# tomka/mitsuba-renderer

Hardware: AMD Instinct MI355X
Metric: Msamples/s (higher is better)
Workload: dtype f32; 1 GPU; C3 1M-tri Cornell: 1024000-tri displaced walls TriMesh + 20480-tri dielectric icosphere + area light, path maxDepth=16 rrDepth=10, 1024x1024, ldsampler 64 spp per GPU (64 per frame, weak scaling), box filter; triangles=1044482, kd_nodes=551229, kd_indices=1101661, parallelism=ImageBlock tiles, morton(tx, ty) % 1 + one RCCL film reduce per frame

## Files before the change

mitsuba-renderer_amd/csrc/api.cpp:

```cpp
#include "host.h"
#include "kernels.h"
#include "devmath.h"
#include "ctx.h"
#include <algorithm>
#include <cstdarg>
#include <cstdio>
#include <cstring>
#include <cstdlib>
#include <cmath>

using namespace mg;

namespace mg {
thread_local std::string g_lastError;

int fail(mtsgpu_ctx *ctx, int code, const char *fmt, ...) {
	char buf[512];
	va_list ap; va_start(ap, fmt); vsnprintf(buf, sizeof(buf), fmt, ap); va_end(ap);
	g_lastError = buf;
	if (ctx) ctx->error = buf;
	return code;
}
}

// ... 41 lines not shown
	c->q.tune_refill = c->tuning.count("refill_min") ? 1u : 0u;
	c->q.tune_batch = (uint32_t) get("batch", 0);
	c->q.tune_dyn_div = (uint32_t) get("dyn_div", 0);
	c->q.tune_blocks_per_cu = (uint32_t) get("blocks_per_cu", 0);
	c->q.tune_plain_below = (uint32_t) get("plain_below", 0);
	c->q.tune_dyn_min_rounds = (uint32_t) get("dyn_min_rounds", 0);
	c->q.bin_hits = c->binHits;
}

int filmWidth(const mtsgpu_ctx *c) { return c->cam.film_width > 0 ? c->cam.film_width : c->cam.width; }
int filmHeight(const mtsgpu_ctx *c) { return c->cam.film_height > 0 ? c->cam.film_height : c->cam.height; }

uint32_t tileMorton(uint32_t tx, uint32_t ty) {
	uint32_t m = 0;
	for (int b = 0; b < 16; ++b)
		m |= ((tx >> b) & 1u) << (2 * b) | ((ty >> b) & 1u) << (2 * b + 1);
	return m;
}

bool samplerHasTables(const mtsgpu_ctx *c) {
	return c->samplerKind == MTSGPU_SAMPLER_LD_KEYED || c->samplerKind == MTSGPU_SAMPLER_STRATIFIED_KEYED;
}

constexpr size_t kBytesPerPath = kPathSlots * 16 + 3 * 16 + (size_t) (kNumBins * (4 + 16) * 5 / 4) + 2 * (4 + 32) + 4 + 4;
uint64_t defaultMaxPaths(mtsgpu_ctx *c) {
	uint64_t paths = 72ull << 20;
	size_t freeB = 0, totalB = 0;
	if (hipMemGetInfo(&freeB, &totalB) == hipSuccess) {
		uint64_t avail = (uint64_t) freeB + (uint64_t) c->pathCap * kBytesPerPath;
		if (c->filmStats && !c->statVar) avail -= std::min<uint64_t>(avail, 16ull * (uint64_t) c->cam.width * (uint64_t) c->cam.height);
		paths = std::min<uint64_t>(paths, std::max<uint64_t>(1ull << 16, avail * 6 / 10 / kBytesPerPath));
	}
	return paths;
}

int ensurePaths(mtsgpu_ctx *c, size_t cap) {
	if (cap <= c->pathCap)
		return 0;
	freeAll(c->pathAllocs);
	c->pathCap = 0;
	cap = (cap + 255) & ~(size_t) 255;
	auto &o = c->pathAllocs;
	int rc = 0;
	rc |= devAlloc(c, &c->paths.base, cap * kPathSlots, o);
	rc |= devAlloc(c, &c->paths.shq_o, cap, o); rc |= devAlloc(c, &c->paths.shq_d, cap, o); rc |= devAlloc(c, &c->paths.shq_nee, cap, o);
	const unsigned gridBlocksMax = c->nCUs * kTraceBlocksPerCuMax;
	const size_t segCap = cap / kBinShards + cap / (4 * kBinShards) + (size_t) kTraceBlock * (gridBlocksMax / kBinShards + 2);
	rc |= devAlloc(c, &c->q.bins_base, segCap * kBinShards * kNumBins, o);
	rc |= devAlloc(c, &c->binHits, segCap * kBinShards * kNumBins, o);
	applyTuning(c);
	c->q.bin_stride = (uint32_t) (segCap * kBinShards);
	if (segCap * kBinShards > 0xFFFFFFFFull) return fail(c, MTSGPU_EINVAL, "pass too large");
	c->q.bin_seg_cap = (uint32_t) segCap;
	rc |= devAlloc(c, &c->queueA, cap, o); rc |= devAlloc(c, &c->queueB, cap, o);
	for (int k = 0; k < 2; ++k) { rc |= devAlloc(c, &c->rayqA[k], cap, o); rc |= devAlloc(c, &c->rayqB[k], cap, o); }
	rc |= devAlloc(c, &c->q.shadow, cap, o);
	rc |= devAlloc(c, &c->counterSets, (size_t) kCounterSets * kNumCounters * kCounterStride, o);
	rc |= devAlloc(c, &c->viewsDev, kNumBins, o);
	rc |= devAlloc(c, &c->devStats, kNumDevStats, o);
	rc |= devAlloc(c, &c->q.trace_counts, kNumTraceCounts, o);
	rc |= devAlloc(c, &c->spillClosest, (size_t) gridBlocksMax * kTraceBlock * trace_spill_levels(), o);
	rc |= devAlloc(c, &c->spillShadow, (size_t) gridBlocksMax * kTraceBlock * trace_spill_levels(), o);
	if (rc) return rc;
	c->q.counters = c->counterSets; c->q.spill = c->spillClosest; c->q.dev_stats = nullptr;
	c->q.spill_stride = gridBlocksMax * kTraceBlock;
	c->q.n_cus = c->nCUs; c->q.force_static = 0;
	applyTuning(c);
	HIPCHK(c, hipMemset(c->q.trace_counts, 0, kNumTraceCounts * sizeof(unsigned long long)));
	c->q.rec = c->q.rec_len = nullptr; c->q.rec_cap = 0;
	c->pathCap = cap;
	return 0;
}

template <typename T> int ensureBuf(mtsgpu_ctx *c, T **p, size_t *cap, size_t need) {
	if (need <= *cap) return 0;
	if (*p) (void) hipFree(*p);
	*p = nullptr; *cap = 0;
	void *raw = nullptr;
	HIPCHK(c, hipMalloc(&raw, need * sizeof(T)));
	*p = static_cast<T *>(raw); *cap = need;
	return 0;
}

int ensureTableWork(mtsgpu_ctx *c, size_t nSlots, uint32_t spp) {
	int rc = ensureBuf(c, &c->ldState, &c->ldStateCap, nSlots); if (rc) return rc;
	return ensureBuf(c, &c->ldScratch, &c->ldScratchCap, ld_table_scratch_entries((uint32_t) nSlots, spp, c->ldDepth));
}

DConfig makeConfig(const mtsgpu_ctx *c, bool slotPerPath) {
	DConfig cfg{};
	std::memcpy(cfg.r2c, c->cam.raster_to_camera, sizeof(cfg.r2c));
	std::memcpy(cfg.c2w, c->cam.camera_to_world, sizeof(cfg.c2w));
	cfg.near_clip = c->cam.near_clip; cfg.far_clip = c->cam.far_clip;
	cfg.aperture_radius = c->cam.aperture_radius; cfg.focus_depth = c->cam.focus_depth; cfg.camera_kind = c->cam.kind;
	cfg.width = c->cam.width; cfg.height = c->cam.height;
	cfg.crop_x = c->cam.crop_offset_x; cfg.crop_y = c->cam.crop_offset_y;
	cfg.pix_w = filmWidth(c); cfg.pix_off = 0;
	cfg.max_depth = c->maxDepth; cfg.rr_depth = c->rrDepth; cfg.strict_normals = c->strictNormals;
	cfg.integrator = c->integrator; cfg.n_lum = c->nLumSamples; cfg.n_bsdf = c->nBsdfSamples;
	cfg.weight_bsdf = 1 / (float) c->nBsdfSamples; cfg.weight_lum = 1 / (float) c->nLumSamples;
	cfg.frac_bsdf = c->nBsdfSamples / (float) (c->nLumSamples + c->nBsdfSamples);
	cfg.frac_lum = c->nLumSamples / (float) (c->nLumSamples + c->nBsdfSamples);
	cfg.sampler_kind = c->samplerKind;
	cfg.spp = effectiveSpp(c); cfg.ld_depth = c->ldDepth; cfg.seed = c->seed;
	cfg.strat_res = 1; while ((uint32_t) cfg.strat_res * (uint32_t) cfg.strat_res < cfg.spp) ++cfg.strat_res;
	cfg.slot_per_path = slotPerPath ? 1 : 0;
// ... 93 lines not shown
			}
			views[b].prefix[kBinShards] = acc;
		}
		if (attempt == 0 && c->tuning.count("test_retry") && c->tuning["test_retry"]) overflow = true;
		if (!overflow) return 0;
		c->stats.bin_overflow_retries++;
	}
	return fail(c, MTSGPU_EHIP, "internal: bin segment overflow with static dealing");
}

int runDirectRounds(mtsgpu_ctx *c, const DConfig &cfg0, uint32_t nPaths, volatile const int *cancel) {
	hipStream_t s = c->stream;
	DConfig cfg = cfg0;
	const size_t counterBytes = kNumCounters * kCounterStride * sizeof(uint32_t);
	auto timedTrace = [&](int mode, bool bin, const uint32_t *queue, uint32_t n, bool coherent) -> int {
		hipEvent_t *ev = c->timeKernels ? nextTraceEvents(c, mode == 1 ? 2 : 0) : nullptr;
		if (ev) HIPCHK(c, hipEventRecord(ev[0], s));
		launch_trace(s, mode, c->countTraversal, bin, c->dsc, c->paths, c->q, queue, n, coherent);
		if (ev) HIPCHK(c, hipEventRecord(ev[1], s));
		HIPCHK(c, hipGetLastError());
		c->stats.trace_launches++;
		return 0;
	};
	HIPCHK(c, hipMemsetAsync(c->q.counters, 0, counterBytes, s));
	c->q.next = c->queueB;
	BinView views[kNumBins];
	RayQueuesOff rqOff{ c };
	rayQueues(c, c->queueA, nullptr);
	int rc = traceAndBin(c, c->queueA, nPaths, true, views); if (rc) return rc;
	rayQueues(c, nullptr, nullptr);
	c->stats.rays_closest += nPaths;
	auto shadeRound = [&](int mode, int index, bool withTerminal) -> int {
		hipEvent_t *sev = c->timeKernels ? nextEventPair(c, c->shadeEvents, c->shadeEvUsed) : nullptr;
		HIPCHK(c, hipMemsetAsync(c->q.counters, 0, counterBytes, s));
		if (sev) HIPCHK(c, hipEventRecord(sev[0], s));
		cfg.dr_mode = mode; cfg.dr_index = index;
		for (int b = 0; b < (withTerminal ? kNumBins : kNumBsdfTypes); ++b)
			launch_shade(s, b, c->dsc, c->paths, cfg, c->q, views[b], nullptr, 0, nullptr, c->dcol, c->dtex, c->dtan);
		if (sev) HIPCHK(c, hipEventRecord(sev[1], s));
		HIPCHK(c, hipGetLastError());
		return readCounters(c);
	};
	for (int j = 0; j < std::max(1, c->nLumSamples); ++j) {
		if (cancel && *cancel) return fail(c, MTSGPU_ECANCEL, "render cancelled");
		rc = shadeRound(1, j, j == 0); if (rc) return rc;
		const uint32_t nShadow = c->hostCounters[kShadowWord];
// ... 30 lines not shown
}

int runBouncesDevice(mtsgpu_ctx *c, const DConfig &cfg, uint32_t nPaths, volatile const int *cancel) {
	hipStream_t s1 = c->stream, s2 = c->stream2;
	const size_t setBytes = (size_t) kNumCounters * kCounterStride * sizeof(uint32_t);
	HIPCHK(c, hipMemsetAsync(c->counterSets, 0, kCounterSets * setBytes, s1));
	c->q.dev_stats = c->devStats;
	c->devStatsUsed = true;
	const int limit = cfg.integrator == 1 ? 2 : (cfg.max_depth > 0 ? cfg.max_depth : 0x7FFFFFFF);
	const int chunk = (int) tuningOr(c, "chunk", 8);
	uint32_t *cur = c->queueA, *nxt = c->queueB;
	uint32_t upper = nPaths;
	bool shadowPending = false;
	int b = 0;
	struct Restore {
		mtsgpu_ctx *c; hipStream_t s2; const bool &pending;
		~Restore() {
			if (pending) (void) hipStreamSynchronize(s2);
			c->q.dev_stats = nullptr; c->q.counters = c->counterSets; c->q.spill = c->spillClosest;
		}
	} restore{ c, s2, shadowPending };
	RayQueuesOff rqOff{ c };
	c->q.nee_parked = tuningOr(c, "nee_parked", 1) != 0 ? 1u : 0u;
	auto timed = [&](std::vector<std::pair<hipEvent_t, hipEvent_t>> &pool, size_t &used, hipStream_t s, int which, int cls = -1) -> int {
		if (!c->timeKernels) return 0;
		hipEvent_t *ev = which == 0 ? (cls >= 0 ? nextTraceEvents(c, cls) : nextEventPair(c, pool, used)) : &pool[used - 1].first;
		if (!ev) return fail(c, MTSGPU_EHIP, "hipEventCreate failed");
		HIPCHK(c, hipEventRecord(ev[which], s));
		return 0;
	};
	while (b < limit && upper > 0) {
		if (cancel && *cancel) return fail(c, MTSGPU_ECANCEL, "render cancelled");
		const int end = (int) std::min<long long>((long long) b + chunk, limit);
		for (; b < end; ++b) {
			uint32_t *set = counterSet(c, b), *prev = counterSet(c, b - 1);
			c->q.counters = set; c->q.next = nxt; c->q.spill = c->spillClosest;
			rayQueues(c, cur, nxt);
			int rc = timed(c->traceEvents, c->traceEvUsed, s1, 0, b == 0 ? 1 : 0); if (rc) return rc;
			launch_trace(s1, 0, c->countTraversal, true, c->dsc, c->paths, c->q, cur, upper, b == 0,
			             b == 0 ? nullptr : prev + (size_t) kNextWord);
			rc = timed(c->traceEvents, c->traceEvUsed, s1, 1); if (rc) return rc;
			if (shadowPending) HIPCHK(c, hipStreamWaitEvent(s1, c->evShadow[(b - 1) & 1], 0));
			rc = timed(c->shadeEvents, c->shadeEvUsed, s1, 0); if (rc) return rc;
			launch_prep(s1, set, prev, c->viewsDev, c->q.bin_seg_cap, c->devStats);
			if (cfg.dr_mode == 0 && tuningOr(c, "shade_fused", 1) != 0) {
				launch_shade_all(s1, c->dsc, c->paths, cfg, c->q, c->viewsDev, c->binMask & kShadeAllBins, upper, c->dcol, c->dtex, c->dtan);
// ... 40 lines not shown
	unsigned long long h[kNumDevStats];
	HIPCHK(c, hipMemcpy(h, c->devStats, sizeof(h), hipMemcpyDeviceToHost));
	c->stats.rays_closest += h[kStatClosest]; c->stats.rays_shadow += h[kStatShadow]; c->stats.trace_launches += h[kStatLaunches];
	if (h[kStatOverflow]) return fail(c, MTSGPU_EHIP, "internal: bin segment overflow in a device-driven frame");
	return 0;
}

int runBounces(mtsgpu_ctx *c, const DConfig &cfg, uint32_t nPaths, volatile const int *cancel) {
	c->q.counters = c->counterSets; c->q.spill = c->spillClosest; c->q.dev_stats = nullptr;
	if (cfg.integrator == 1 && (cfg.n_lum > 1 || cfg.n_bsdf > 1))
		return runDirectRounds(c, cfg, nPaths, cancel);
	{
		const long sf = tuningOr(c, "sync_free", -1);
		if (sf == 1 || (sf < 0 && nPaths <= (8u << 20)))
			return runBouncesDevice(c, cfg, nPaths, cancel);
	}
	uint32_t nQ = nPaths;
	uint32_t *cur = c->queueA, *nxt = c->queueB;
	bool first = true;
	hipStream_t s = c->stream;
	const size_t setBytes = (size_t) kNumCounters * kCounterStride * sizeof(uint32_t);
	RayQueuesOff rqOff{ c };
	c->q.nee_parked = tuningOr(c, "nee_parked", 1) != 0 ? 1u : 0u;
	for (int b = 0; nQ > 0; ++b) {
		if (cancel && *cancel)
			return fail(c, MTSGPU_ECANCEL, "render cancelled");
		c->q.counters = counterSet(c, b); c->q.spill = c->spillClosest;
		HIPCHK(c, hipMemsetAsync(c->q.counters, 0, setBytes, s));
		c->q.next = nxt;
		rayQueues(c, cur, nxt);
		BinView views[kNumBins];
		int rc = traceAndBin(c, cur, nQ, first, views); if (rc) return rc;
		c->stats.rays_closest += nQ;
		hipEvent_t *sev = c->timeKernels ? nextEventPair(c, c->shadeEvents, c->shadeEvUsed) : nullptr;
		if (sev) HIPCHK(c, hipEventRecord(sev[0], s));
		for (int bin = 0; bin < kNumBins; ++bin)
			launch_shade(s, bin, c->dsc, c->paths, cfg, c->q, views[bin], nullptr, 0, nullptr, c->dcol, c->dtex, c->dtan);
		if (sev) HIPCHK(c, hipEventRecord(sev[1], s));
		HIPCHK(c, hipGetLastError());
		rc = readCounters(c); if (rc) return rc;
		const uint32_t nNext = c->hostCounters[kNextWord], nShadow = c->hostCounters[kShadowWord];
		if (nShadow) {
			DQueues q2 = c->q; q2.spill = c->spillShadow;
			c->lastPass.shadowMax = std::max(c->lastPass.shadowMax, nShadow);
			hipEvent_t *ev2 = c->timeKernels ? nextTraceEvents(c, 2) : nullptr;
			if (ev2) HIPCHK(c, hipEventRecord(ev2[0], s));
// ... 135 lines not shown
		    || hipMemcpy(c->primes, primes.data(), primes.size() * sizeof(uint16_t), hipMemcpyHostToDevice) != hipSuccess) {
			mtsgpu_destroy(c); return fail(nullptr, MTSGPU_EHIP, "prime table upload failed");
		}
	}
	*out = c;
	return 0;
}

void mtsgpu_destroy(mtsgpu_ctx *c) {
	if (!c) return;
	(void) hipSetDevice(c->device);
	(void) hipDeviceSynchronize();
	freeAll(c->sceneAllocs); freeAll(c->colorAllocs); freeAll(c->texAllocs); freeAll(c->pathAllocs);
	if (c->ownFilm && c->film) (void) hipFree(c->film);
	if (c->pixelList) (void) hipFree(c->pixelList);
	if (c->ldScr) (void) hipFree(c->ldScr);
	if (c->ldPerm) (void) hipFree(c->ldPerm);
	if (c->ldState) (void) hipFree(c->ldState);
	if (c->ldScratch) (void) hipFree(c->ldScratch);
	if (c->arrScr) (void) hipFree(c->arrScr);
	if (c->arrPerm) (void) hipFree(c->arrPerm);
	if (c->arrPts) (void) hipFree(c->arrPts);
	if (c->primSave) (void) hipFree(c->primSave);
	if (c->primes) (void) hipFree(c->primes);
	if (c->pathLen) (void) hipFree(c->pathLen);
	if (c->explicitSamples) (void) hipFree(c->explicitSamples);
	if (c->filtValues) (void) hipFree(c->filtValues);
	if (c->statVar) (void) hipFree(c->statVar);
	if (c->statN) (void) hipFree(c->statN);
	if (c->tileMeta) (void) hipFree(c->tileMeta);
	if (c->blocks) (void) hipFree(c->blocks);
	if (c->hostCounters) (void) hipHostFree(c->hostCounters);
	for (auto &e : c->traceEvents) { (void) hipEventDestroy(e.first); (void) hipEventDestroy(e.second); }
	for (auto &e : c->shadeEvents) { (void) hipEventDestroy(e.first); (void) hipEventDestroy(e.second); }
	if (c->ownStream && c->stream) (void) hipStreamDestroy(c->stream);
	if (c->stream2) (void) hipStreamDestroy(c->stream2);
	for (hipEvent_t e : { c->evShade[0], c->evShade[1], c->evShadow[0], c->evShadow[1], c->evCount }) if (e) (void) hipEventDestroy(e);
	delete c;
}

int mtsgpu_set_stream(mtsgpu_ctx *c, void *hip_stream) {
	if (!c) return fail(nullptr, MTSGPU_EINVAL, "null context");
	if (c->ownStream && c->stream) { (void) hipStreamSynchronize(c->stream); (void) hipStreamDestroy(c->stream); }
	if (hip_stream) { c->stream = (hipStream_t) hip_stream; c->ownStream = false; }
	else { HIPCHK(c, hipStreamCreate(&c->stream)); c->ownStream = true; }
	return 0;
// ... 882 lines not shown
	hipEvent_t e0 = nullptr, e1 = nullptr;
	auto cleanup = [&]() {
		for (uint32_t *p : { rec, recLen, order, tr, batchLen, sink }) if (p) (void) hipFree(p);
		if (tmp) (void) hipFree(tmp);
		if (e0) (void) hipEventDestroy(e0);
		if (e1) (void) hipEventDestroy(e1);
		c->q.rec = c->q.rec_len = nullptr; c->q.rec_cap = 0;
	};
	#define RR_CHK(expr) do { hipError_t e_ = (expr); if (e_ != hipSuccess) { cleanup(); \
		return fail(c, MTSGPU_EHIP, "%s failed: %s (%s:%d)", #expr, hipGetErrorString(e_), __FILE__, __LINE__); } } while (0)
	RR_CHK(hipMalloc((void **) &rec, (size_t) n * cap * 4)); RR_CHK(hipMalloc((void **) &recLen, (size_t) n * 4));
	RR_CHK(hipMalloc((void **) &order, (size_t) n * 4)); RR_CHK(hipMalloc((void **) &tr, (size_t) nBatches * cap * 64 * 4));
	RR_CHK(hipMalloc((void **) &batchLen, (size_t) nBatches * 4)); RR_CHK(hipMalloc((void **) &sink, 4));
	RR_CHK(hipEventCreate(&e0)); RR_CHK(hipEventCreate(&e1));
	const size_t counterBytes = kNumCounters * kCounterStride * sizeof(uint32_t);
	c->q.counters = c->counterSets; c->q.spill = mode == 1 ? c->spillShadow : c->spillClosest; c->q.dev_stats = nullptr;
	c->q.next = c->queueB;
	if (kind == 1) {
		launch_generate(s, c->dsc, c->paths, lp.cfg, c->pixelList + lp.base, lp.nSlots, nullptr, lp.nPaths, c->queueA);
		RR_CHK(hipGetLastError());
		c->lastPass.valid = false;
	}
	if (kind == 2) {
		RR_CHK(hipMalloc((void **) &tmp, (size_t) n * 3 * sizeof(float4)));
		launch_gather_strided(s, tmp, c->paths.shq_o, n, stride); launch_gather_strided(s, tmp + n, c->paths.shq_d, n, stride);
		launch_gather_strided(s, tmp + 2 * (size_t) n, c->paths.shq_nee, n, stride);
		RR_CHK(hipMemcpyAsync(c->paths.shq_o, tmp, (size_t) n * sizeof(float4), hipMemcpyDeviceToDevice, s));
		RR_CHK(hipMemcpyAsync(c->paths.shq_d, tmp + n, (size_t) n * sizeof(float4), hipMemcpyDeviceToDevice, s));
		RR_CHK(hipMemcpyAsync(c->paths.shq_nee, tmp + 2 * (size_t) n, (size_t) n * sizeof(float4), hipMemcpyDeviceToDevice, s));
		c->lastPass.shadowMax = 0;
	} else {
		launch_iota_strided(s, c->queueA, n, stride);
		launch_gather_strided(s, c->rayqA[0], c->paths.base + 0, n, stride * kPathSlots);
		launch_gather_strided(s, c->rayqA[1], c->paths.base + 1, n, stride * kPathSlots);
		rayQueues(c, c->queueA, nullptr);
	}
	RayQueuesOff rqOff{ c };
	const uint32_t *queue = mode == 1 ? c->q.shadow : c->queueA;
	RR_CHK(hipMemsetAsync(recLen, 0, (size_t) n * 4, s));
	RR_CHK(hipMemsetAsync(c->q.trace_counts, 0, kNumTraceCounts * sizeof(unsigned long long), s));
	RR_CHK(hipMemsetAsync(c->q.counters, 0, counterBytes, s));
	c->q.rec = rec; c->q.rec_len = recLen; c->q.rec_cap = cap;
	launch_trace(s, mode, true, bin, c->dsc, c->paths, c->q, queue, n, coherent);
	c->q.rec = c->q.rec_len = nullptr; c->q.rec_cap = 0;
	RR_CHK(hipGetLastError());
	std::vector<uint32_t> len(n);
	RR_CHK(hipMemcpyAsync(len.data(), recLen, (size_t) n * 4, hipMemcpyDeviceToHost, s));
	RR_CHK(hipStreamSynchronize(s));
	unsigned long long cnt[kNumTraceCounts];
	RR_CHK(hipMemcpy(cnt, c->q.trace_counts, sizeof(cnt), hipMemcpyDeviceToHost));
	std::vector<uint32_t> ord(n), first(cap + 2, 0u);
	unsigned long long total = 0, truncated = 0;
	for (uint32_t i = 0; i < n; ++i) { const uint32_t l = std::min(len[i], cap); total += l; if (len[i] > cap) ++truncated; first[cap - l + 1]++; }
	for (uint32_t l = 0; l <= cap; ++l) first[l + 1] += first[l];
	for (uint32_t i = 0; i < n; ++i) ord[first[cap - std::min(len[i], cap)]++] = i;
	RR_CHK(hipMemcpyAsync(order, ord.data(), (size_t) n * 4, hipMemcpyHostToDevice, s));
	launch_build_replay(s, rec, recLen, order, n, cap, tr, batchLen);
	RR_CHK(hipGetLastError());
	float prodMs = 1e30f, replayMs = 1e30f;
	for (int i = 0; i <= reps; ++i) {
// ... 543 lines not shown
```

mitsuba-renderer_amd/csrc/ctx.h:

```cpp
#pragma once
#include "host.h"
#include "kernels.h"
#include <map>
#include <string>
#include <utility>
#include <vector>

struct mtsgpu_ctx {
	int device = 0;
	uint32_t nCUs = 256;
	hipStream_t stream = nullptr;
	bool ownStream = false;
	hipStream_t stream2 = nullptr;
	hipEvent_t evShade[2] = { nullptr, nullptr }, evShadow[2] = { nullptr, nullptr }, evCount = nullptr;
	std::string error;

	bool haveScene = false;
	mg::DScene dsc{};
	std::vector<void *> sceneAllocs;
	uint32_t nTris = 0;
	struct HostScene {
		uint32_t nVerts = 0;
		std::vector<uint32_t> triIdx, shapeTriOffset, shapeType, bsdfType;
		std::vector<int32_t> shapeBsdf;
// ... 21 lines not shown
	bool hqEdges = false;
	int integrator = 0, nLumSamples = 1, nBsdfSamples = 1;
	float *filtValues = nullptr;
	bool filmStats = false;
	float *statVar = nullptr; uint32_t *statN = nullptr; size_t statPixels = 0;
	int statsForm = -1;
	mg::TileMeta *tileMeta = nullptr; size_t tileMetaCap = 0;
	float *blocks = nullptr; size_t blocksCap = 0;

	size_t pathCap = 0;
	mg::DPaths paths{};
	mg::DQueues q{};
	uint32_t *queueA = nullptr, *queueB = nullptr;
	float4 *rayqA[2] = { nullptr, nullptr }, *rayqB[2] = { nullptr, nullptr };
	uint4 *binHits = nullptr;
	uint32_t *pixelList = nullptr; size_t pixelListCap = 0;
	std::vector<uint32_t> renderPixels; std::vector<mg::TileMeta> renderTiles;
	std::vector<long long> renderKey; bool renderListValid = false;
	uint32_t *ldScr = nullptr; uint16_t *ldPerm = nullptr; size_t ldScrCap = 0, ldPermCap = 0;
	uint16_t *ldScratch = nullptr; size_t ldScratchCap = 0;
	unsigned long long *ldState = nullptr; size_t ldStateCap = 0;
	uint32_t *arrScr = nullptr; uint16_t *arrPerm = nullptr; float2 *arrPts = nullptr; size_t arrScrCap = 0, arrPermCap = 0, arrPtsCap = 0;
	float4 *primSave = nullptr; size_t primSaveCap = 0;
	uint16_t *primes = nullptr;
	uint32_t *explicitSamples = nullptr; size_t explicitCap = 0;
	uint32_t *hostCounters = nullptr;
	uint32_t *counterSets = nullptr;
	uint32_t *spillClosest = nullptr, *spillShadow = nullptr;
	mg::BinView *viewsDev = nullptr;
	unsigned long long *devStats = nullptr;
	bool devStatsUsed = false;
	uint32_t binMask = 0x1FFu;
	unsigned long long *pathLen = nullptr;
	std::vector<void *> pathAllocs;

	mtsgpu_stats stats{};
	std::vector<std::pair<hipEvent_t, hipEvent_t>> traceEvents, shadeEvents;
	size_t traceEvUsed = 0, shadeEvUsed = 0;
	std::vector<unsigned char> traceEvClass;
	struct LastPass { bool valid = false; mg::DConfig cfg{}; size_t base = 0; uint32_t nSlots = 0, nPaths = 0, shadowMax = 0; } lastPass;
};


namespace mg {
extern thread_local std::string g_lastError;
int fail(mtsgpu_ctx *ctx, int code, const char *fmt, ...);
// ... 5 lines not shown
```

mitsuba-renderer_amd/csrc/shade_path.h:

```cpp
#pragma once
#include "shade_bsdf.h"

namespace mg {

#ifndef MG_SHADE_PACKED
#define MG_SHADE_PACKED 0
#endif
constexpr int kRowStride = MG_SHADE_PACKED ? kPathSlots : kPathSlots + 1;
struct ShadeRow {
	float4 *base; uint32_t x;
	__device__ __forceinline__ float4 &operator[](int k) const { return base[MG_SHADE_PACKED ? ((uint32_t) k ^ x) : (uint32_t) k]; }
};
__device__ __forceinline__ uint32_t shade_row_index(uint32_t lane, uint32_t k) { return lane * kRowStride + (MG_SHADE_PACKED ? (k ^ (lane & 7u)) : k); }

template <int BT, bool ROUNDS, bool SKY, int VCOL, bool TAN = false>
__device__ __forceinline__ void shade_path(const DScene &sc, const DPaths &ps, const DConfig &cfg, const uint32_t id,
                                           const float4 ro, const float4 rd, const uint4 h, const float4 T4, const float4 L4,
                                           const ShadeRow row, bool &continues, bool &wantShadow, V3 &neeV, V3 &shO, V3 &shD, const DColors &col,
                                           const DTextures &tex, const DTangents &tan = DTangents{ nullptr, nullptr }) {
	{
		const int mode = ROUNDS ? cfg.dr_mode : 0;
		const bool skipToNee = ROUNDS && mode == 1 && cfg.dr_index > 0, skipToBsdf = ROUNDS && mode == 2;
		const V3 rayO(ro.x, ro.y, ro.z), rayD(rd.x, rd.y, rd.z);
		const bool valid = h.w != kNoPrim;
// ... 258 lines not shown
				h = reinterpret_cast<const uint4 &>(ps.prim[3 * (size_t) id + 2]);
			} else if (cfg.n_bsdf > 1) {
				ps.prim[3 * (size_t) id] = ro; ps.prim[3 * (size_t) id + 1] = rd;
				ps.prim[3 * (size_t) id + 2] = reinterpret_cast<const float4 &>(h);
			}
		}
	}
	__builtin_amdgcn_fence(__ATOMIC_ACQ_REL, "wavefront"); __builtin_amdgcn_wave_barrier();
	{
		const uint32_t prim = h.w;
		const uint64_t validMask = __ballot(active && prim != kNoPrim);
		const uint32_t sub4 = lane_id() & 3u, grp4 = lane_id() >> 2;
		const uint32_t slotOf = sub4 < 2u ? sub4 : sub4 + 1u;
		#pragma unroll
		for (int r = 0; r < 4; ++r) {
			const uint32_t src = grp4 + 16u * r;
			const uint32_t sprim = (uint32_t) __shfl((int) prim, (int) src);
			if ((validMask >> src) & 1ull) rows[shade_row_index(src, slotOf)] = sc.tri_pos[(size_t) sprim * kTriStride + sub4];
		}
	}
	__builtin_amdgcn_fence(__ATOMIC_ACQ_REL, "wavefront"); __builtin_amdgcn_wave_barrier();
	if (active)
		shade_path<BT, ROUNDS, SKY, VCOL, TAN>(sc, ps, cfg, id, ro, rd, h, T4, L4, row, continues, wantShadow, neeV, shO, shD, col, tex, tan);
	__builtin_amdgcn_fence(__ATOMIC_ACQ_REL, "wavefront"); __builtin_amdgcn_wave_barrier();
	#pragma unroll
	for (int r = 0; r < 8; ++r) {
		const uint32_t src = grp + 8u * r;
		const uint32_t sid = (uint32_t) __shfl((int) id, (int) src);
		if ((actMask >> src) & 1ull) st_stream<4>(&ps.base[(size_t) sid * kPathSlots + sub], rows[shade_row_index(src, sub)]);
	}

	const uint32_t wave = threadIdx.x >> 6, lane = lane_id();
	const unsigned long long mN = __ballot(continues), mS = __ballot(wantShadow);
	if (lane == 0) { s_cnt[0][wave] = (uint32_t) __popcll(mN); s_cnt[1][wave] = (uint32_t) __popcll(mS); }
	__syncthreads();
	if (threadIdx.x < 2) {
		uint32_t total = 0;
		for (int w = 0; w < kShadeBlock / 64; ++w) total += s_cnt[threadIdx.x][w];
		s_base[threadIdx.x] = total ? atomicAdd(&q.counters[threadIdx.x == 0 ? kNextWord : kShadowWord], total) : 0u;
	}
	__syncthreads();
	uint32_t offN = s_base[0], offS = s_base[1];
	for (uint32_t w = 0; w < wave; ++w) { offN += s_cnt[0][w]; offS += s_cnt[1][w]; }
	const unsigned long long below = (1ull << lane) - 1ull;
	if (continues) {
		const uint32_t pos = offN + (uint32_t) __popcll(mN & below);
		q.next[pos] = id;
		if (ps.rqn_o) {
			st_stream<4>(&ps.rqn_o[pos], rows[shade_row_index(lane, 0)]);
			st_stream<4>(&ps.rqn_d[pos], rows[shade_row_index(lane, 1)]);
		}
	}
	if (wantShadow) {
		const uint32_t pos = offS + (uint32_t) __popcll(mS & below);
		st_stream<4>(&ps.shq_o[pos], make_float4(shO.x, shO.y, shO.z, 0.0f));
		st_stream<4>(&ps.shq_d[pos], make_float4(shD.x, shD.y, shD.z, 0.0f));
		st_stream<4>(&ps.shq_nee[pos], make_float4(neeV.x, neeV.y, neeV.z, __uint_as_float(id)));
	}
}

template <int BT, bool ROUNDS, bool SKY>
__global__ MG_SHADE_BOUNDS void k_shade(DScene sc, DPaths ps, DConfig cfg, DQueues q, BinView view_host,
                                                       const BinView *views_dev, const uint32_t *bin_ids) {
	__shared__ ShadeShared sh;
	shade_block<BT, ROUNDS, SKY, kSlotBlock>(sc, ps, cfg, q, views_dev ? views_dev[BT].prefix : view_host.prefix, bin_ids, blockIdx.x, sh, DColors{ nullptr, nullptr });
}
template <int BT, bool ROUNDS, bool SKY>
__global__ MG_SHADE_BOUNDS void k_shade_vcol(DScene sc, DPaths ps, DConfig cfg, DQueues q, BinView view_host,
                                                            const BinView *views_dev, const uint32_t *bin_ids, DColors col) {
	__shared__ ShadeShared sh;
	shade_block<BT, ROUNDS, SKY, kSlotColor>(sc, ps, cfg, q, views_dev ? views_dev[BT].prefix : view_host.prefix, bin_ids, blockIdx.x, sh, col);
}
template <int BT, bool ROUNDS, bool SKY>
__global__ MG_SHADE_BOUNDS void k_shade_tex(DScene sc, DPaths ps, DConfig cfg, DQueues q, BinView view_host,
                                                           const BinView *views_dev, const uint32_t *bin_ids, DColors col, DTextures tex) {
	__shared__ ShadeShared sh;
	shade_block<BT, ROUNDS, SKY, kSlotTexture>(sc, ps, cfg, q, views_dev ? views_dev[BT].prefix : view_host.prefix, bin_ids, blockIdx.x, sh, col, tex);
}
template <int BT, bool ROUNDS, bool SKY>
__global__ MG_SHADE_BOUNDS void k_shade_tan(DScene sc, DPaths ps, DConfig cfg, DQueues q, BinView view_host,
// ... 58 lines not shown
```

mitsuba-renderer_amd/csrc/trace.hip:

```cpp
#include "kdevice.h"

namespace mg {


__device__ __forceinline__ uint32_t lanes_below(uint64_t mask) {
	return __builtin_amdgcn_mbcnt_hi((uint32_t) (mask >> 32), __builtin_amdgcn_mbcnt_lo((uint32_t) mask, 0u));
}
size_t trace_spill_levels() { return kSpillLevels; }
size_t trace_stack_levels() { return kStackLDS + kSpillLevels; }
uint32_t trace_top_nodes() { return kTopNodes; }

__device__ __forceinline__ const uint4 *leaf_head(const DTraceScene &sc, uint32_t e) { return &sc.leaf_ta[kLeafStride * (size_t) e]; }
__device__ __forceinline__ const uint4 *leaf_tail(const DTraceScene &sc, uint32_t e, uint32_t half) { return &sc.leaf_ta[kLeafStride * (size_t) e + 1 + half]; }

template <int MODE, bool COUNT, bool BIN>
__device__ __forceinline__ void trace_body(const DTraceScene &sc, const DPaths &ps, const DQueues &q, const TracePlan &plan,
                                           const uint32_t *queue, uint32_t n, const uint32_t first, const uint32_t stride,
                                           uint32_t (*s_stack)[kTraceBlock], uint32_t (*s_mbox)[kTraceBlock], const uint4 *s_top) {
	uint32_t g_pair = 0, l_pair = 0, g_node = 0, l_node = 0, g_tail = 0, g_spill = 0, g_head = 0;
	uint32_t rec_n = 0, rec_slot = 0;
	auto rec_add = [&](uint32_t kind, uint32_t idx) {
		if (COUNT && q.rec) {
			if (rec_n < q.rec_cap) q.rec[(size_t) rec_slot * q.rec_cap + rec_n] = (kind << 29) | idx;
			rec_n++;
		}
	};
	auto load_node = [&](uint32_t i) -> uint2 {
		if (kTopPairs && i < 2u * kTopPairs) { if (COUNT) l_node++; return reinterpret_cast<const uint2 *>(s_top)[i]; }
		if (COUNT) { g_node++; rec_add(kReqNode, i); }
		return sc.nodes[i];
	};
	auto load_pair = [&](uint32_t left) -> uint4 {
		if (kTopPairs && left < 2u * kTopPairs) { if (COUNT) l_pair++; return s_top[left >> 1]; }
		if (COUNT) { g_pair++; rec_add(kReqPair, left >> 1); }
		return reinterpret_cast<const uint4 *>(sc.nodes)[left >> 1];
	};
	constexpr bool kMbox = MODE == 0 || COUNT;
	const uint32_t tid = threadIdx.x;
// ... 57 lines not shown
						}
					}
				}
				if (BIN) {
					uint32_t cnt = 0, rank = 0;
					#pragma unroll
					for (int b = 0; b < kNumBins; ++b) {
						const uint64_t m = __builtin_amdgcn_ballot_w64(bin == b);
						if (lane == (uint32_t) b) cnt = (uint32_t) __popcll(m);
						if (bin == b) rank = lanes_below(m);
					}
					uint32_t base = 0;
					if (lane < (uint32_t) kNumBins && cnt != 0u)
						base = atomicAdd(&q.counters[(lane * kBinShards + shard) * kCounterStride], cnt);
					base = __shfl(base, bin < 0 ? 0 : bin);
					const uint32_t pos = base + rank;
					if (bin >= 0 && pos < q.bin_seg_cap) {
						const size_t at = (size_t) bin * q.bin_stride + (size_t) shard * q.bin_seg_cap + pos;
						st_stream<1>(&q.bins_base[at], id);
						if (hitsToBins) st_stream<1>(&q.bin_hits[at], make_uint4(__float_as_uint(best_t), __float_as_uint(best_u), __float_as_uint(best_v), best_prim));
					}
				}
			} else if (MODE == 1) {
				if (done && !found) {
					const float4 c = ps.shq_nee[id];
					const uint32_t pid = __float_as_uint(c.w);
					if (q.nee_parked) {
						ps.slot(pid, 2) = make_float4(c.x, c.y, c.z, __uint_as_float(kNeeTag));
					} else {
						float4 L = ps.Li(pid);
						L.x += c.x; L.y += c.y; L.z += c.z;
						ps.Li(pid) = L;
					}
				}
			} else {
				if (done)
					ps.hit(id) = make_uint4(0u, 0u, 0u, found ? 1u : 0u);
			}
			done = false;
			if (remaining == 0u)
				break;

			const uint32_t r = lanes_below(~liveMask & limitMask);
			const bool take = !has && lane < B && r < remaining;
			const uint32_t taken = (B - nlive < remaining) ? B - nlive : remaining;
			const uint32_t my = sup_base + r;
			sup_base += taken; sup_left -= taken;
			MG_WSLOT(w_batch);
			if (take) {
				id = (MODE == 1) ? my : ld_stream<1>(&queue[my]);
				if (COUNT && q.rec) { rec_slot = my; rec_n = 0; if (MODE != 1 && !(MODE == 0 && ps.rq_o)) { rec_add(kReqRay, id * kPathSlots); rec_add(kReqRay, id * kPathSlots + 1); } }
				float4 a, b;
				float rmint, rmaxt;
				if (MODE == 1) {
					a = ld_stream<1>(&ps.shq_o[my]); b = ld_stream<1>(&ps.shq_d[my]);
					rmint = kShadowEpsilon; rmaxt = 1 - kShadowEpsilon;
				} else {
					if (MODE == 0 && ps.rq_o) { a = ld_stream<1>(&ps.rq_o[my]); b = ld_stream<1>(&ps.rq_d[my]); }
					else { a = ld_stream<1>(&ps.ray_o(id)); b = ld_stream<1>(&ps.ray_d(id)); }
					rmint = a.w; rmaxt = b.w;
				}
				ox = a.x; oy = a.y; oz = a.z; dx = b.x; dy = b.y; dz = b.z;
				rx = 1.0f / dx; ry = 1.0f / dy; rz = 1.0f / dz;
				bool go = true;
				mint = -MG_INF; maxt = MG_INF;
				#pragma unroll
				for (int i = 0; i < 3; ++i) {
					const float direction = sel3(dx, dy, dz, i), origin = sel3(ox, oy, oz, i);
					const float minVal = sc.aabb_min[i], maxVal = sc.aabb_max[i];
					if (direction == 0) {
						if (origin < minVal || origin > maxVal) go = false;
					} else {
						const float rc = sel3(rx, ry, rz, i);
						float t1 = (minVal - origin) * rc, t2 = (maxVal - origin) * rc;
						if (t1 > t2) { const float tmp = t1; t1 = t2; t2 = tmp; }
						mint = smax(mint, t1);
						maxt = smin(maxt, t2);
						if (mint > maxt) go = false;
					}
// ... 165 lines not shown
				}
				if (finished) {
					has = false; done = true; found = (MODE == 0) ? (best_prim != kNoPrim) : hitShadow;
					if (COUNT && q.rec) { if (MODE != 1 && !(MODE == 0 && BIN)) rec_add(kReqHit, id * kPathSlots + 2); q.rec_len[rec_slot] = rec_n; }
				}
				}
			}
		}
	}

	if (COUNT) {
		unsigned long long v[16] = { c_inner, c_leaf, c_idx, c_tri, w_inner, w_leaf, w_outer, w_batch, g_pair, l_pair, g_node, l_node, g_tail, g_spill, g_head, c_tail_out };
		#pragma unroll
		for (int k = 0; k < 16; ++k) {
			unsigned long long x = v[k];
			for (int off = 32; off > 0; off >>= 1)
				x += __shfl_down(x, off);
			if (lane == 0)
				atomicAdd(&q.trace_counts[k], x);
		}
	}
}

template <int MODE, bool COUNT, bool BIN>
__global__ __launch_bounds__(kTraceBlock, trace_waves_per_simd(MODE)) void k_trace(DTraceScene sc, DPaths ps, DQueues q,
                                                          const uint32_t *queue, uint32_t n_host, const uint32_t *n_dev) {
	__shared__ uint32_t s_stack[kStackLDS][kTraceBlock];
	__shared__ uint32_t s_mbox[(MODE == 0 || COUNT) ? 8 : 1][kTraceBlock];
	__shared__ uint4 s_top[kTopPairs ? kTopPairs : 1];
	const uint32_t n = n_dev ? (uint32_t) __builtin_amdgcn_readfirstlane((int) *n_dev) : n_host;
	const TracePlan plan = trace_plan(n, MODE, q);
	if (blockIdx.x >= plan.blocks)
		return;
	if (q.dev_stats && blockIdx.x == 0 && threadIdx.x == 0) {
		atomicAdd(&q.dev_stats[MODE == 0 ? kStatClosest : kStatShadow], (unsigned long long) n);
		atomicAdd(&q.dev_stats[kStatLaunches], 1ull);
	}
	const uint32_t first = (blockIdx.x * (kTraceBlock / 64u) + (threadIdx.x >> 6)) * plan.batch;
	const uint32_t stride = plan.blocks * (kTraceBlock / 64u) * plan.batch;
	if (kTopPairs) {
		for (uint32_t t = threadIdx.x; t < kTopPairs; t += kTraceBlock) s_top[t] = reinterpret_cast<const uint4 *>(sc.nodes)[t];
		__syncthreads();
	}
	trace_body<MODE, COUNT, BIN>(sc, ps, q, plan, queue, n, first, stride, s_stack, s_mbox, s_top);
}

__global__ __launch_bounds__(256) void k_prep(const uint32_t *cur, uint32_t *next_set, BinView *views, uint32_t bin_seg_cap,
                                              unsigned long long *dev_stats) {
	__shared__ uint32_t s_cnt[kNumBins * kBinShards];
	const uint32_t t = threadIdx.x;
	if (t < (uint32_t) (kNumBins * kBinShards)) {
		const uint32_t c = cur[t * kCounterStride];
		s_cnt[t] = c;
		if (c > bin_seg_cap && dev_stats) atomicAdd(&dev_stats[kStatOverflow], 1ull);
	}
	if (t < (uint32_t) kNumCounters) next_set[t * kCounterStride] = 0u;
	__syncthreads();
	if (t < (uint32_t) kNumBins) {
		uint32_t acc = 0;
		for (int k = 0; k < kBinShards; ++k) {
			views[t].prefix[k] = acc;
			const uint32_t c = s_cnt[t * kBinShards + k];
			acc += c < bin_seg_cap ? c : bin_seg_cap;
		}
		views[t].prefix[kBinShards] = acc;
	}
}

template <int MODE, bool COUNT, bool BIN>
static void launch_trace_t(hipStream_t s, const DScene &sc, const DPaths &ps, const DQueues &q, const uint32_t *queue, uint32_t n,
                           const uint32_t *n_dev) {
	unsigned blocks = trace_plan(n, MODE, q).blocks;
	if (n_dev) {
		const unsigned minBatch = (q.tune_batch >= 1 && q.tune_batch <= 64) ? q.tune_batch : (q.coherent ? 64u : 8u);
		unsigned perCu = trace_blocks_per_cu(MODE);
		if (q.tune_blocks_per_cu && q.tune_blocks_per_cu < perCu) perCu = q.tune_blocks_per_cu;
		blocks = std::min<unsigned>(blocks_for(n, minBatch * (kTraceBlock / 64)), q.n_cus * perCu);
	}
	if (!blocks) return;
	hipLaunchKernelGGL((k_trace<MODE, COUNT, BIN>), dim3(blocks), dim3(kTraceBlock), 0, s, trace_scene(sc), ps, q, queue, n, n_dev);
}

void launch_trace(hipStream_t s, int mode, bool count, bool bin, const DScene &sc, const DPaths &ps,
                  const DQueues &q, const uint32_t *queue, uint32_t n, bool coherent, const uint32_t *n_dev) {
	if (!n) return;
	DQueues qq = q;
	qq.coherent = coherent ? 1u : 0u;
	if (n_dev)
		qq.force_static = 1u;
	if (mode == 0) {
		if (bin) { if (count) launch_trace_t<0, true, true>(s, sc, ps, qq, queue, n, n_dev); else launch_trace_t<0, false, true>(s, sc, ps, qq, queue, n, n_dev); }
		else     { if (count) launch_trace_t<0, true, false>(s, sc, ps, qq, queue, n, n_dev); else launch_trace_t<0, false, false>(s, sc, ps, qq, queue, n, n_dev); }
	} else if (mode == 1) {
		if (count) launch_trace_t<1, true, false>(s, sc, ps, qq, queue, n, n_dev); else launch_trace_t<1, false, false>(s, sc, ps, qq, queue, n, n_dev);
	} else {
		if (count) launch_trace_t<2, true, false>(s, sc, ps, qq, queue, n, n_dev); else launch_trace_t<2, false, false>(s, sc, ps, qq, queue, n, n_dev);
	}
}

void launch_prep(hipStream_t s, const uint32_t *cur, uint32_t *next_set, BinView *views_dev, uint32_t bin_seg_cap,
                 unsigned long long *dev_stats) {
	hipLaunchKernelGGL(k_prep, dim3(1), dim3(256), 0, s, cur, next_set, views_dev, bin_seg_cap, dev_stats);
}

}
```

Measured before the change: 300.6 Msamples/s.

## Park NEE contribution in path slot and drop per-shadow-ray NEE queue

In parked mode the shade kernel now writes the NEE radiance directly into the path's slot 2, and stores the path id in the shadow-origin w component. The shadow trace then only clears that slot when the ray is occluded, instead of reading the separate shq_nee buffer and writing the slot on a miss. This removes one float4 store per shadow ray in shading and one float4 load per unoccluded shadow ray in tracing, and frees a per-path buffer so more paths fit. The trade-off is an extra slot write for every shadow-requesting path, occluded or not. The shq_nee buffer is now allocated lazily, only when non-parked mode is used.

```diff
diff --git a/mitsuba-renderer_amd/csrc/api.cpp b/mitsuba-renderer_amd/csrc/api.cpp
--- a/mitsuba-renderer_amd/csrc/api.cpp
+++ b/mitsuba-renderer_amd/csrc/api.cpp
@@ -87,7 +87,7 @@
 	return c->samplerKind == MTSGPU_SAMPLER_LD_KEYED || c->samplerKind == MTSGPU_SAMPLER_STRATIFIED_KEYED;
 }
 
-constexpr size_t kBytesPerPath = kPathSlots * 16 + 3 * 16 + (size_t) (kNumBins * (4 + 16) * 5 / 4) + 2 * (4 + 32) + 4 + 4;
+constexpr size_t kBytesPerPath = kPathSlots * 16 + 2 * 16 + (size_t) (kNumBins * (4 + 16) * 5 / 4) + 2 * (4 + 32) + 4 + 4;
 uint64_t defaultMaxPaths(mtsgpu_ctx *c) {
 	uint64_t paths = 72ull << 20;
 	size_t freeB = 0, totalB = 0;
@@ -108,7 +108,7 @@
 	auto &o = c->pathAllocs;
 	int rc = 0;
 	rc |= devAlloc(c, &c->paths.base, cap * kPathSlots, o);
-	rc |= devAlloc(c, &c->paths.shq_o, cap, o); rc |= devAlloc(c, &c->paths.shq_d, cap, o); rc |= devAlloc(c, &c->paths.shq_nee, cap, o);
+	rc |= devAlloc(c, &c->paths.shq_o, cap, o); rc |= devAlloc(c, &c->paths.shq_d, cap, o);
 	const unsigned gridBlocksMax = c->nCUs * kTraceBlocksPerCuMax;
 	const size_t segCap = cap / kBinShards + cap / (4 * kBinShards) + (size_t) kTraceBlock * (gridBlocksMax / kBinShards + 2);
 	rc |= devAlloc(c, &c->q.bins_base, segCap * kBinShards * kNumBins, o);
@@ -147,6 +147,12 @@
 	return 0;
 }
 
+int ensureNeeQueue(mtsgpu_ctx *c) {
+	int rc = ensureBuf(c, &c->shqNee, &c->shqNeeCap, c->pathCap);
+	c->paths.shq_nee = c->shqNee;
+	return rc;
+}
+
 int ensureTableWork(mtsgpu_ctx *c, size_t nSlots, uint32_t spp) {
 	int rc = ensureBuf(c, &c->ldState, &c->ldStateCap, nSlots); if (rc) return rc;
 	return ensureBuf(c, &c->ldScratch, &c->ldScratchCap, ld_table_scratch_entries((uint32_t) nSlots, spp, c->ldDepth));
@@ -286,6 +292,7 @@
 		c->stats.trace_launches++;
 		return 0;
 	};
+	{ int rc = ensureNeeQueue(c); if (rc) return rc; }
 	HIPCHK(c, hipMemsetAsync(c->q.counters, 0, counterBytes, s));
 	c->q.next = c->queueB;
 	BinView views[kNumBins];
@@ -362,6 +369,7 @@
 	} restore{ c, s2, shadowPending };
 	RayQueuesOff rqOff{ c };
 	c->q.nee_parked = tuningOr(c, "nee_parked", 1) != 0 ? 1u : 0u;
+	if (!c->q.nee_parked) { int rc = ensureNeeQueue(c); if (rc) return rc; }
 	auto timed = [&](std::vector<std::pair<hipEvent_t, hipEvent_t>> &pool, size_t &used, hipStream_t s, int which, int cls = -1) -> int {
 		if (!c->timeKernels) return 0;
 		hipEvent_t *ev = which == 0 ? (cls >= 0 ? nextTraceEvents(c, cls) : nextEventPair(c, pool, used)) : &pool[used - 1].first;
@@ -448,6 +456,7 @@
 	const size_t setBytes = (size_t) kNumCounters * kCounterStride * sizeof(uint32_t);
 	RayQueuesOff rqOff{ c };
 	c->q.nee_parked = tuningOr(c, "nee_parked", 1) != 0 ? 1u : 0u;
+	if (!c->q.nee_parked) { int rc = ensureNeeQueue(c); if (rc) return rc; }
 	for (int b = 0; nQ > 0; ++b) {
 		if (cancel && *cancel)
 			return fail(c, MTSGPU_ECANCEL, "render cancelled");
@@ -629,6 +638,7 @@
 	if (c->arrPerm) (void) hipFree(c->arrPerm);
 	if (c->arrPts) (void) hipFree(c->arrPts);
 	if (c->primSave) (void) hipFree(c->primSave);
+	if (c->shqNee) (void) hipFree(c->shqNee);
 	if (c->primes) (void) hipFree(c->primes);
 	if (c->pathLen) (void) hipFree(c->pathLen);
 	if (c->explicitSamples) (void) hipFree(c->explicitSamples);
@@ -1557,12 +1567,10 @@
 		c->lastPass.valid = false;
 	}
 	if (kind == 2) {
-		RR_CHK(hipMalloc((void **) &tmp, (size_t) n * 3 * sizeof(float4)));
+		RR_CHK(hipMalloc((void **) &tmp, (size_t) n * 2 * sizeof(float4)));
 		launch_gather_strided(s, tmp, c->paths.shq_o, n, stride); launch_gather_strided(s, tmp + n, c->paths.shq_d, n, stride);
-		launch_gather_strided(s, tmp + 2 * (size_t) n, c->paths.shq_nee, n, stride);
 		RR_CHK(hipMemcpyAsync(c->paths.shq_o, tmp, (size_t) n * sizeof(float4), hipMemcpyDeviceToDevice, s));
 		RR_CHK(hipMemcpyAsync(c->paths.shq_d, tmp + n, (size_t) n * sizeof(float4), hipMemcpyDeviceToDevice, s));
-		RR_CHK(hipMemcpyAsync(c->paths.shq_nee, tmp + 2 * (size_t) n, (size_t) n * sizeof(float4), hipMemcpyDeviceToDevice, s));
 		c->lastPass.shadowMax = 0;
 	} else {
 		launch_iota_strided(s, c->queueA, n, stride);
@@ -1571,6 +1579,7 @@
 		rayQueues(c, c->queueA, nullptr);
 	}
 	RayQueuesOff rqOff{ c };
+	c->q.nee_parked = mode == 1 ? 1u : 0u;
 	const uint32_t *queue = mode == 1 ? c->q.shadow : c->queueA;
 	RR_CHK(hipMemsetAsync(recLen, 0, (size_t) n * 4, s));
 	RR_CHK(hipMemsetAsync(c->q.trace_counts, 0, kNumTraceCounts * sizeof(unsigned long long), s));
diff --git a/mitsuba-renderer_amd/csrc/ctx.h b/mitsuba-renderer_amd/csrc/ctx.h
--- a/mitsuba-renderer_amd/csrc/ctx.h
+++ b/mitsuba-renderer_amd/csrc/ctx.h
@@ -67,6 +67,7 @@
 	unsigned long long *ldState = nullptr; size_t ldStateCap = 0;
 	uint32_t *arrScr = nullptr; uint16_t *arrPerm = nullptr; float2 *arrPts = nullptr; size_t arrScrCap = 0, arrPermCap = 0, arrPtsCap = 0;
 	float4 *primSave = nullptr; size_t primSaveCap = 0;
+	float4 *shqNee = nullptr; size_t shqNeeCap = 0;
 	uint16_t *primes = nullptr;
 	uint32_t *explicitSamples = nullptr; size_t explicitCap = 0;
 	uint32_t *hostCounters = nullptr;
diff --git a/mitsuba-renderer_amd/csrc/shade_path.h b/mitsuba-renderer_amd/csrc/shade_path.h
--- a/mitsuba-renderer_amd/csrc/shade_path.h
+++ b/mitsuba-renderer_amd/csrc/shade_path.h
@@ -304,6 +304,7 @@
 	__builtin_amdgcn_fence(__ATOMIC_ACQ_REL, "wavefront"); __builtin_amdgcn_wave_barrier();
 	if (active)
 		shade_path<BT, ROUNDS, SKY, VCOL, TAN>(sc, ps, cfg, id, ro, rd, h, T4, L4, row, continues, wantShadow, neeV, shO, shD, col, tex, tan);
+	if (q.nee_parked && wantShadow) row[2] = make_float4(neeV.x, neeV.y, neeV.z, __uint_as_float(kNeeTag));
 	__builtin_amdgcn_fence(__ATOMIC_ACQ_REL, "wavefront"); __builtin_amdgcn_wave_barrier();
 	#pragma unroll
 	for (int r = 0; r < 8; ++r) {
@@ -335,9 +336,9 @@
 	}
 	if (wantShadow) {
 		const uint32_t pos = offS + (uint32_t) __popcll(mS & below);
-		st_stream<4>(&ps.shq_o[pos], make_float4(shO.x, shO.y, shO.z, 0.0f));
+		st_stream<4>(&ps.shq_o[pos], make_float4(shO.x, shO.y, shO.z, __uint_as_float(id)));
 		st_stream<4>(&ps.shq_d[pos], make_float4(shD.x, shD.y, shD.z, 0.0f));
-		st_stream<4>(&ps.shq_nee[pos], make_float4(neeV.x, neeV.y, neeV.z, __uint_as_float(id)));
+		if (!q.nee_parked) st_stream<4>(&ps.shq_nee[pos], make_float4(neeV.x, neeV.y, neeV.z, __uint_as_float(id)));
 	}
 }
 
diff --git a/mitsuba-renderer_amd/csrc/trace.hip b/mitsuba-renderer_amd/csrc/trace.hip
--- a/mitsuba-renderer_amd/csrc/trace.hip
+++ b/mitsuba-renderer_amd/csrc/trace.hip
@@ -13,7 +13,7 @@
 __device__ __forceinline__ const uint4 *leaf_head(const DTraceScene &sc, uint32_t e) { return &sc.leaf_ta[kLeafStride * (size_t) e]; }
 __device__ __forceinline__ const uint4 *leaf_tail(const DTraceScene &sc, uint32_t e, uint32_t half) { return &sc.leaf_ta[kLeafStride * (size_t) e + 1 + half]; }
 
-template <int MODE, bool COUNT, bool BIN>
+template <int MODE, bool COUNT, bool BIN, bool PARKED>
 __device__ __forceinline__ void trace_body(const DTraceScene &sc, const DPaths &ps, const DQueues &q, const TracePlan &plan,
                                            const uint32_t *queue, uint32_t n, const uint32_t first, const uint32_t stride,
                                            uint32_t (*s_stack)[kTraceBlock], uint32_t (*s_mbox)[kTraceBlock], const uint4 *s_top) {
@@ -117,16 +117,14 @@
 					}
 				}
 			} else if (MODE == 1) {
-				if (done && !found) {
+				if (PARKED) {
+					if (done && found) ps.slot(id, 2) = make_float4(0.0f, 0.0f, 0.0f, 0.0f);
+				} else if (done && !found) {
 					const float4 c = ps.shq_nee[id];
 					const uint32_t pid = __float_as_uint(c.w);
-					if (q.nee_parked) {
-						ps.slot(pid, 2) = make_float4(c.x, c.y, c.z, __uint_as_float(kNeeTag));
-					} else {
-						float4 L = ps.Li(pid);
-						L.x += c.x; L.y += c.y; L.z += c.z;
-						ps.Li(pid) = L;
-					}
+					float4 L = ps.Li(pid);
+					L.x += c.x; L.y += c.y; L.z += c.z;
+					ps.Li(pid) = L;
 				}
 			} else {
 				if (done)
@@ -150,6 +148,7 @@
 				if (MODE == 1) {
 					a = ld_stream<1>(&ps.shq_o[my]); b = ld_stream<1>(&ps.shq_d[my]);
 					rmint = kShadowEpsilon; rmaxt = 1 - kShadowEpsilon;
+					if (PARKED) id = __float_as_uint(a.w);
 				} else {
 					if (MODE == 0 && ps.rq_o) { a = ld_stream<1>(&ps.rq_o[my]); b = ld_stream<1>(&ps.rq_d[my]); }
 					else { a = ld_stream<1>(&ps.ray_o(id)); b = ld_stream<1>(&ps.ray_d(id)); }
@@ -361,7 +360,7 @@
 	}
 }
 
-template <int MODE, bool COUNT, bool BIN>
+template <int MODE, bool COUNT, bool BIN, bool PARKED = false>
 __global__ __launch_bounds__(kTraceBlock, trace_waves_per_simd(MODE)) void k_trace(DTraceScene sc, DPaths ps, DQueues q,
                                                           const uint32_t *queue, uint32_t n_host, const uint32_t *n_dev) {
 	__shared__ uint32_t s_stack[kStackLDS][kTraceBlock];
@@ -381,7 +380,7 @@
 		for (uint32_t t = threadIdx.x; t < kTopPairs; t += kTraceBlock) s_top[t] = reinterpret_cast<const uint4 *>(sc.nodes)[t];
 		__syncthreads();
 	}
-	trace_body<MODE, COUNT, BIN>(sc, ps, q, plan, queue, n, first, stride, s_stack, s_mbox, s_top);
+	trace_body<MODE, COUNT, BIN, PARKED>(sc, ps, q, plan, queue, n, first, stride, s_stack, s_mbox, s_top);
 }
 
 __global__ __launch_bounds__(256) void k_prep(const uint32_t *cur, uint32_t *next_set, BinView *views, uint32_t bin_seg_cap,
@@ -406,7 +405,7 @@
 	}
 }
 
-template <int MODE, bool COUNT, bool BIN>
+template <int MODE, bool COUNT, bool BIN, bool PARKED = false>
 static void launch_trace_t(hipStream_t s, const DScene &sc, const DPaths &ps, const DQueues &q, const uint32_t *queue, uint32_t n,
                            const uint32_t *n_dev) {
 	unsigned blocks = trace_plan(n, MODE, q).blocks;
@@ -417,7 +416,7 @@
 		blocks = std::min<unsigned>(blocks_for(n, minBatch * (kTraceBlock / 64)), q.n_cus * perCu);
 	}
 	if (!blocks) return;
-	hipLaunchKernelGGL((k_trace<MODE, COUNT, BIN>), dim3(blocks), dim3(kTraceBlock), 0, s, trace_scene(sc), ps, q, queue, n, n_dev);
+	hipLaunchKernelGGL((k_trace<MODE, COUNT, BIN, PARKED>), dim3(blocks), dim3(kTraceBlock), 0, s, trace_scene(sc), ps, q, queue, n, n_dev);
 }
 
 void launch_trace(hipStream_t s, int mode, bool count, bool bin, const DScene &sc, const DPaths &ps,
@@ -431,7 +430,8 @@
 		if (bin) { if (count) launch_trace_t<0, true, true>(s, sc, ps, qq, queue, n, n_dev); else launch_trace_t<0, false, true>(s, sc, ps, qq, queue, n, n_dev); }
 		else     { if (count) launch_trace_t<0, true, false>(s, sc, ps, qq, queue, n, n_dev); else launch_trace_t<0, false, false>(s, sc, ps, qq, queue, n, n_dev); }
 	} else if (mode == 1) {
-		if (count) launch_trace_t<1, true, false>(s, sc, ps, qq, queue, n, n_dev); else launch_trace_t<1, false, false>(s, sc, ps, qq, queue, n, n_dev);
+		if (qq.nee_parked) { if (count) launch_trace_t<1, true, false, true>(s, sc, ps, qq, queue, n, n_dev); else launch_trace_t<1, false, false, true>(s, sc, ps, qq, queue, n, n_dev); }
+		else               { if (count) launch_trace_t<1, true, false>(s, sc, ps, qq, queue, n, n_dev); else launch_trace_t<1, false, false>(s, sc, ps, qq, queue, n, n_dev); }
 	} else {
 		if (count) launch_trace_t<2, true, false>(s, sc, ps, qq, queue, n, n_dev); else launch_trace_t<2, false, false>(s, sc, ps, qq, queue, n, n_dev);
 	}
```

Result: faster. 306.0 Msamples/s, median of 6 (+1.8%).
